# arneschneuing/DiffSBDD

Hardware: NVIDIA H100
Metric: ligand_atoms_per_sec_500step_ddpm (higher is better)
Workload: dtype f32

## Files before the change

### diffsbdd_b200/csrc/dsb_tc.cu

```cuda
#include "dsb_tc.cuh"

namespace dsb {
using namespace tc;

__global__ void pack_b_image_kernel(float* __restrict__ hi, float* __restrict__ lo, const float* __restrict__ src, int lds,
                                    int scol, int n_rows, int n_dst_off, int K, int chunks, int TN) {
  const int64_t idx = (int64_t)blockIdx.x * blockDim.x + threadIdx.x;
  if (idx >= (int64_t)n_rows * K) return;
  const int n = (int)(idx / K), k = (int)(idx - (int64_t)n * K);
  const int nd = n_dst_off + n, nt = nd / TN, nl = nd % TN;
  const int kc = k / TKC, c = (k % TKC) >> 2, j = k & 3;
  const size_t off = ((size_t)nt * chunks + kc) * (size_t)(TN * TKC) + sw128_offset(nl, c) / 4 + j;
  const float w = src[(size_t)n * lds + scol + k];
  const float h = tf32_hi(w);
  hi[off] = h;
  lo[off] = w - h;
}

void launch_pack_b_image(float* hi, float* lo, const float* src, int lds, int scol, int n_rows, int n_dst_off, int K, int tn) {
  const int64_t tot = (int64_t)n_rows * K;
  pack_b_image_kernel<<<(unsigned)((tot + 255) / 256), 256>>>(hi, lo, src, lds, scol, n_rows, n_dst_off, K, K / TKC, tn);
}

__global__ void pack_b_image_f16_kernel(__half* __restrict__ hi, __half* __restrict__ lo, const float* __restrict__ src, int lds,
                                        int scol, int n_rows, int n_dst_off, int K, int chunks, float scale, int TN) {
  const int64_t idx = (int64_t)blockIdx.x * blockDim.x + threadIdx.x;
  if (idx >= (int64_t)n_rows * K) return;
  const int n = (int)(idx / K), k = (int)(idx - (int64_t)n * K);
  const int nd = n_dst_off + n, nt = nd / TN, nl = nd % TN;
  const int kc = k / TKC16, c16 = (k % TKC16) >> 3, j = k & 7;
  const size_t off = ((size_t)nt * chunks + kc) * (size_t)(TN * 64) + sw128_offset(nl, c16) / 2 + j;
  const float w = src[(size_t)n * lds + scol + k] * scale;
  const __half h = __float2half_rn(w);
  hi[off] = h;
  lo[off] = __float2half_rn(w - __half2float(h));
}

void launch_pack_b_image_f16(float* hi, float* lo, const float* src, int lds, int scol, int n_rows, int n_dst_off, int K, float scale, int tn) {
  const int64_t tot = (int64_t)n_rows * K;
  pack_b_image_f16_kernel<<<(unsigned)((tot + 255) / 256), 256>>>(reinterpret_cast<__half*>(hi), reinterpret_cast<__half*>(lo), src,
                                                                  lds, scol, n_rows, n_dst_off, K, K / TKC16, scale, tn);
}

__global__ void absmax_kernel(const float* __restrict__ src, int lds, int scol, int n_rows, int K, unsigned* __restrict__ out) {
  const int64_t idx = (int64_t)blockIdx.x * blockDim.x + threadIdx.x;
  float v = 0.f;
  if (idx < (int64_t)n_rows * K) { const int n = (int)(idx / K), k = (int)(idx - (int64_t)n * K); v = fabsf(src[(size_t)n * lds + scol + k]); }
#pragma unroll
  for (int o = 16; o > 0; o >>= 1) v = fmaxf(v, __shfl_xor_sync(0xffffffffu, v, o));
  if ((threadIdx.x & 31) == 0) atomicMax(out, __float_as_uint(v));
}
void launch_absmax(const float* src, int lds, int scol, int n_rows, int K, unsigned* out) {
  const int64_t tot = (int64_t)n_rows * K;
  absmax_kernel<<<(unsigned)((tot + 255) / 256), 256>>>(src, lds, scol, n_rows, K, out);
}

constexpr size_t kControlBytes = 128;
static_assert(sizeof(Control) <= kControlBytes, "Control block grew");
__device__ __forceinline__ char* align1024(uint8_t* raw) {
  return reinterpret_cast<char*>(raw) + ((1024u - (smem_u32(raw) & 1023u)) & 1023u);
}
template <int H> constexpr size_t tc_smem_base() { return 1024 + (size_t)NSTAGE * Geo<H>::STAGE_BYTES + kControlBytes; }

struct TcGemmArgs {
  const float* A1; int lda1; int K1;
  const float* A2; int lda2; int K2; float div2; const int32_t* deg2;
  const float* Bhi; const float* Blo;
  const float* bias; const float* R; int ldr;
  float* C; int ldc; int M; int Nn; int act;
  float* Z; int ldz;
  int dead_mt; int dead_nt;
  float inv_scale;
};

struct TileMap {
  int ntn, ntm, dead_mt, dead_nt, nA, n_live;
  __device__ TileMap(int M, int Nn, int dmt, int dnt, int TN) {
    ntn = Nn / TN; ntm = (M + TM - 1) / TM;
    dead_nt = dnt; dead_mt = dnt > 0 ? (dmt < ntm ? dmt : ntm) : ntm;
    nA = dead_mt * ntn;
    n_live = nA + (ntm - dead_mt) * (ntn - dead_nt);
  }
  __device__ void get(int t, int& mt, int& nt) const {
    if (t < nA) { mt = t / ntn; nt = t - mt * ntn; }
    else { const int u = t - nA, w = ntn - dead_nt; mt = dead_mt + u / w; nt = dead_nt + (u - (u / w) * w); }
  }
};

template <TcFormat FMT, int H>
__global__ void __launch_bounds__(TC_THREADS, 1) tc_node_gemm_kernel(TcGemmArgs g) {
  using G = Geo<H>;
  constexpr bool F16 = FMT != TcFormat::TF32x3;
  constexpr int TN = H, HPC = F16 ? 2 : 1;
  extern __shared__ uint8_t smem_raw[];
  char* const stages = align1024(smem_raw);
  Control* ctl = reinterpret_cast<Control*>(stages + NSTAGE * G::STAGE_BYTES);
  const int wg = threadIdx.x >> 7, warp = (threadIdx.x >> 5) & 3, lane = threadIdx.x & 31;
  const TileMap tm(g.M, g.Nn, g.dead_mt, g.dead_nt, TN);
  const int n_tiles = tm.n_live;
  const int n_my = ((int)blockIdx.x < n_tiles) ? (n_tiles - (int)blockIdx.x + (int)gridDim.x - 1) / (int)gridDim.x : 0;
  if (n_my == 0) return;
  const int K = g.K1 + g.K2, chunks = K / (F16 ? TKC16 : TKC);
  const uint32_t total = (uint32_t)(n_my * chunks);
  pdl_trigger();
  if (threadIdx.x == 0) control_init(ctl);
  __syncthreads();
  pdl_wait();
  const WeightStream<FMT, H> wst{ctl, stages};
  auto issue_w = [&](uint32_t q) {
    const int it = (int)(q / chunks), kc = (int)(q - (uint32_t)it * chunks);
    int mt, nt;
    tm.get(blockIdx.x + it * gridDim.x, mt, nt);
    const size_t off = ((size_t)nt * chunks + kc) * G::B_CHUNK_FLOATS;
    wst.issue(q, g.Bhi + off, g.Blo + off);
  };
  if (threadIdx.x >= MMA_THREADS) {
    regs_dec<WEIGHT_WG_REGS>();
    if (threadIdx.x == MMA_THREADS)
      for (uint32_t q = 0; q < total; ++q) issue_w(q);
    return;
  }
  regs_inc<MMA_WG_REGS>();

  const int sr = lane >> 3, pc = lane & 7;
  const int r0 = wg * WG_ROWS + 16 * warp + 4 * sr;
  const int re = wg * WG_ROWS + 16 * warp + (lane >> 2);
  const bool divides = g.div2 != 1.0f || g.deg2 != nullptr;
  float acc[G::ACC];
  MmaTracker trk;
// ... 27 lines not shown
          }
          store_pair<FMT>(st + piece_offset<F16>(r0 + i, hf, pc), pk2(x.x, x.y), pk2(x.z, x.w));
        }
      }
      fence_proxy_async();
      wg_sync(wg);
      mbar_wait(&ctl->full_w[s], (q >> 1) & 1);
      wgmma_fence();
      mma_chunk<FMT, H>(acc, st, wg, kc == 0);
      wgmma_commit();
      trk.release_prev(ctl, (int)q, lane == 0);
    }
    trk.drain<H>(ctl, acc, lane == 0);
    const f32x2 ip = pk2(g.inv_scale, g.inv_scale);
#pragma unroll
    for (int j = 0; j < H / 8; ++j) {
      const int n = n0 + 8 * j + 2 * (lane & 3);
      const f32x2 b = g.bias ? *reinterpret_cast<const float2*>(g.bias + n) : pk2(0.f, 0.f);
#pragma unroll
      for (int hh = 0; hh < 2; ++hh) {
        f32x2 x = pk2(acc[4 * j + 2 * hh], acc[4 * j + 2 * hh + 1]);
        x = F16 ? fma2(x, ip, b) : add2(x, b);
        if (g.act == 1) x = silu2(x);
        upk2(x, acc[4 * j + 2 * hh], acc[4 * j + 2 * hh + 1]);
      }
    }
    if (g.R) {
#pragma unroll
      for (int j = 0; j < H / 8; ++j) {
        const int n = n0 + 8 * j + 2 * (lane & 3);
#pragma unroll
        for (int hh = 0; hh < 2; ++hh) {
          const int row = min(m0 + re + 8 * hh, g.M - 1);
          const f32x2 x = add2(*reinterpret_cast<const float2*>(g.R + (size_t)row * g.ldr + n),
                               pk2(acc[4 * j + 2 * hh], acc[4 * j + 2 * hh + 1]));
          upk2(x, acc[4 * j + 2 * hh], acc[4 * j + 2 * hh + 1]);
        }
      }
    }
    acc_fence(acc);
#pragma unroll
    for (int j = 0; j < H / 8; ++j) {
      const int n = n0 + 8 * j + 2 * (lane & 3);
#pragma unroll
      for (int hh = 0; hh < 2; ++hh) {
        const int row = m0 + re + 8 * hh;
        if (row < g.M) {
          *reinterpret_cast<float2*>(g.C + (size_t)row * g.ldc + n) = pk2(acc[4 * j + 2 * hh], acc[4 * j + 2 * hh + 1]);
          if (g.Z) *reinterpret_cast<float2*>(g.Z + (size_t)row * g.ldz + n) = make_float2(0.f, 0.f);
        }
      }
    }
  }
}

struct EdgeScalars {
  float d2[TM], d0[TM];
  int row[TM], col[TM], type[TM];
  float dir[3][TM];
};

template <int H>
struct EdgeExtra {
  float vec[2][3 * H];
  float wa[H];
  EdgeScalars sc[2];
};

struct TcEdgeArgs {
  const float* P; int ldp;
  const float4* x; const float4* cent; const int32_t* gid;
  const int32_t* vrow_ptr; const int32_t* vmap; int n_rows;
  const int32_t *erow, *ecol; const float* ed0; int NL;
  int nm;
  const float* W2hi[2]; const float* W2lo[2];
  const float* wr[2]; const float* wr0[2]; const float* tb[2]; const float* b2[2];
  const float* wa; const float* ba;
  float norm_constant, coords_range; int use_tanh;
  float* agg;
  float4* xagg;
  float inv_scale[2];
  float* part;
  int vcap;
};

template <bool COORD>
struct ScalarSteps {
  int e, r, c, gi;
  float d0;
  float4 xi, xj;
  __device__ __forceinline__ void step(int k, const TcEdgeArgs& a, EdgeScalars* sc, int pr, int v0, int V, int m) {
    if (k == 0) {
      const int vr = v0 + pr;
      e = a.vmap[min(vr, V - 1)];
      e = vr < V ? e : -1;
    } else if (k == 1) {
      const int ec = max(e, 0);
      r = a.erow[ec]; c = a.ecol[ec]; d0 = a.ed0[ec];
      r = e >= 0 ? r : 0; c = e >= 0 ? c : 0;
    } else if (k == 2) {
      xi = a.x[r]; xj = a.x[c];
      if (COORD) gi = a.gid[r];
    } else {
      const bool live = e >= 0;
      const float dx = xi.x - xj.x, dy = xi.y - xj.y, dz = xi.z - xj.z;
      const float d2 = dx * dx + dy * dy + dz * dz;
// ... 232 lines not shown
          t = live ? t : 0.f;
          t += __shfl_xor_sync(0xffffffffu, t, 4);
          t += __shfl_xor_sync(0xffffffffu, t, 8);
          tr[k] = t;
        }
        const int crow = hh ? crow_hi : crow_lo;
        if constexpr (DET) {
          if (chunk_lane && (lane & 3) == 0)
            reinterpret_cast<float4*>(a.part)[(size_t)((e0 + (r & ~3)) / kRowChunk) * nm + m] = make_float4(tr[0], tr[1], tr[2], 0.f);
        } else if (chunk_lane && (lane & 3) == 0 && crow >= 0) {
#pragma unroll
          for (int k = 0; k < 3; ++k) atomicAdd(reinterpret_cast<float*>(a.xagg) + (size_t)crow * 4 + k, tr[k]);
        }
      }
    }
    m = m_next; e0 = e0_next;
  }
}

template <int H> static size_t gemm_smem_bytes() { return tc_smem_base<H>(); }
template <int H> static size_t edge_smem_bytes() {
  static_assert(tc_smem_base<H>() + sizeof(EdgeExtra<H>) <= 232448, "edge kernel exceeds the 227 KB of shared memory per CTA");
  return tc_smem_base<H>() + sizeof(EdgeExtra<H>);
}

bool tc_width_supported(int H) { return H == 128 || H == 192 || H == 256; }

template <typename Fn>
static int dispatch_width(int H, Fn&& fn) {
  switch (H) {
    case 128: return fn.template operator()<128>();
    case 192: return fn.template operator()<192>();
    case 256: return fn.template operator()<256>();
    default: set_error("tensor-core kernels exist for hidden_nf 128, 192, 256 (got %d)", H); return DSB_ERR_UNSUPPORTED_CONFIG;
  }
}

template <typename Fn>
static int dispatch_tc(TcFormat f, int H, Fn&& fn) {
  return dispatch_width(H, [&]<int W>() -> int {
    switch (f) {
      case TcFormat::TF32x3: return fn.template operator()<TcFormat::TF32x3, W>();
      case TcFormat::F16x3: return fn.template operator()<TcFormat::F16x3, W>();
      default: return fn.template operator()<TcFormat::F16x1, W>();
    }
  });
}

int configure_tc_kernels(int H) {
  for (const TcFormat f : {TcFormat::TF32x3, TcFormat::F16x3, TcFormat::F16x1}) {
    const int e = dispatch_tc(f, H, [&]<TcFormat F, int W>() -> int {
      const int gs = (int)gemm_smem_bytes<W>(), es = (int)edge_smem_bytes<W>();
      DSB_CUDA_OK(cudaFuncSetAttribute(tc_node_gemm_kernel<F, W>, cudaFuncAttributeMaxDynamicSharedMemorySize, gs));
      DSB_CUDA_OK(cudaFuncSetAttribute(tc_edge_kernel<false, F, W, false>, cudaFuncAttributeMaxDynamicSharedMemorySize, es));
      DSB_CUDA_OK(cudaFuncSetAttribute(tc_edge_kernel<false, F, W, true>, cudaFuncAttributeMaxDynamicSharedMemorySize, es));
      DSB_CUDA_OK(cudaFuncSetAttribute(tc_edge_kernel<true, F, W, false>, cudaFuncAttributeMaxDynamicSharedMemorySize, es));
      DSB_CUDA_OK(cudaFuncSetAttribute(tc_edge_kernel<true, F, W, true>, cudaFuncAttributeMaxDynamicSharedMemorySize, es));
      DSB_CUDA_OK(cudaFuncSetAttribute(tc_edge_kernel<false, F, W, false, true>, cudaFuncAttributeMaxDynamicSharedMemorySize, es));
      DSB_CUDA_OK(cudaFuncSetAttribute(tc_edge_kernel<false, F, W, true, true>, cudaFuncAttributeMaxDynamicSharedMemorySize, es));
      DSB_CUDA_OK(cudaFuncSetAttribute(tc_edge_kernel<true, F, W, false, true>, cudaFuncAttributeMaxDynamicSharedMemorySize, es));
      DSB_CUDA_OK(cudaFuncSetAttribute(tc_edge_kernel<true, F, W, true, true>, cudaFuncAttributeMaxDynamicSharedMemorySize, es));
      return 0;
    });
    if (e) return e;
  }
  return 0;
}

int launch_tc_node_gemm(const dsb_dynamics* d, const GemmArgs& g, const TcImage& w, int n_tile_off, TcFormat fmt, int32_t* status,
                        cudaStream_t s) {
  (void)status;
  if (g.M == 0) return 0;
  const bool f16 = fmt != TcFormat::TF32x3;
  const int K = g.K1 + g.K2, TN = d->cfg.hidden_nf;
  if ((g.Nn % TN) || (K % TKC16) || (g.K1 % TKC16) || (g.lda1 % 4) || (g.ldc % 4)) {
    set_error("tc_node_gemm: unsupported shape K1=%d K2=%d Nn=%d", g.K1, g.K2, g.Nn);
    return DSB_ERR_INVALID_ARGUMENT;
  }
  TcGemmArgs a;
  a.A1 = g.A1; a.lda1 = g.lda1; a.K1 = g.K1; a.A2 = g.A2; a.lda2 = g.lda2; a.K2 = g.K2; a.div2 = g.div2; a.deg2 = g.deg2;
  const size_t img_off = (size_t)n_tile_off * (K / (f16 ? TKC16 : TKC)) * (size_t)(TN * TKC);
  a.Bhi = (f16 ? w.h_hi : w.t_hi) + img_off; a.Blo = (f16 ? w.h_lo : w.t_lo) + img_off;
  a.Z = g.Z; a.ldz = g.ldz;
  a.dead_nt = g.dead_cols / TN; a.dead_mt = a.dead_nt > 0 ? (g.dead_rows_from + TM - 1) / TM : 0;
  a.bias = g.bias; a.R = g.R; a.ldr = g.ldr; a.C = g.C; a.ldc = g.ldc; a.M = g.M; a.Nn = g.Nn; a.act = g.act;
  a.inv_scale = f16 ? w.h_inv : 1.0f;
  const int ntn_ = g.Nn / TN, ntm_ = (g.M + TM - 1) / TM;
  const int dmt_ = a.dead_nt > 0 ? (a.dead_mt < ntm_ ? a.dead_mt : ntm_) : ntm_;
  const int n_tiles = dmt_ * ntn_ + (ntm_ - dmt_) * (ntn_ - a.dead_nt);
  const int grid = n_tiles < d->num_sms ? n_tiles : d->num_sms;
  return dispatch_tc(fmt, TN, [&]<TcFormat F, int W>() -> int {
    DSB_CUDA_OK(launch_k(tc_node_gemm_kernel<F, W>, grid, TC_THREADS, gemm_smem_bytes<W>(), s, a));
    return 0;
  });
}

int launch_tc_edge_gcl(const dsb_dynamics* d, const Dims& dm, const Workspace& ws, const GclW& w, const float4* x, PView pv, TcFormat fmt,
                       int32_t* status, cudaStream_t s) {
  (void)status;
  const bool f16 = fmt != TcFormat::TF32x3;
  TcEdgeArgs a = {};
  a.P = pv.P; a.ldp = pv.ldp; a.x = x; a.cent = ws.cent; a.gid = ws.gid; a.vrow_ptr = ws.vrow_ptr; a.vmap = ws.vmap; a.n_rows = dm.N;
  a.erow = ws.erow; a.ecol = ws.ecol; a.ed0 = ws.ed0; a.NL = dm.NL; a.nm = 1;
  a.W2hi[0] = f16 ? w.iW2.h_hi : w.iW2.t_hi; a.W2lo[0] = f16 ? w.iW2.h_lo : w.iW2.t_lo;
  a.inv_scale[0] = f16 ? w.iW2.h_inv : 1.0f; a.inv_scale[1] = 1.0f;
  a.wr[0] = w.wr; a.wr0[0] = w.wr0; a.tb[0] = w.tb; a.b2[0] = w.b2;
  a.wa = w.wa; a.ba = w.ba; a.agg = ws.agg; a.part = ws.part; a.vcap = ws.vcap;
  const bool det = d->deterministic != 0;
  return dispatch_tc(fmt, d->cfg.hidden_nf, [&]<TcFormat F, int W>() -> int {
    auto kern = w.tb ? tc_edge_kernel<false, F, W, true> : tc_edge_kernel<false, F, W, false>;
    if (det) kern = w.tb ? tc_edge_kernel<false, F, W, true, true> : tc_edge_kernel<false, F, W, false, true>;
    DSB_CUDA_OK(launch_k(kern, d->num_sms, TC_THREADS, edge_smem_bytes<W>(), s, a));
    return 0;
  });
}

int launch_tc_edge_coord(const dsb_dynamics* d, const Dims& dm, const Workspace& ws, const EquivW& w, const float4* x, PView pv, TcFormat fmt,
                         int32_t* status, cudaStream_t s) {
  (void)status;
  const bool f16 = fmt != TcFormat::TF32x3;
  const dsb_config& c = d->cfg;
  TcEdgeArgs a = {};
  a.nm = c.reflection_equivariant ? 1 : 2;
  a.P = pv.P; a.ldp = pv.ldp; a.x = x; a.cent = ws.cent; a.gid = ws.gid; a.vrow_ptr = ws.vrow_ptr; a.vmap = ws.vmap; a.n_rows = dm.n_coord_rows;
  a.erow = ws.erow; a.ecol = ws.ecol; a.ed0 = ws.ed0; a.NL = dm.NL;
  a.inv_scale[0] = a.inv_scale[1] = 1.0f;
  for (int m = 0; m < a.nm; ++m) {
    a.W2hi[m] = f16 ? w.iW2[m].h_hi : w.iW2[m].t_hi; a.W2lo[m] = f16 ? w.iW2[m].h_lo : w.iW2[m].t_lo;
    a.inv_scale[m] = f16 ? w.iW2[m].h_inv : 1.0f;
    a.wr[m] = w.wr[m]; a.wr0[m] = w.wr0[m]; a.tb[m] = w.tb[m]; a.b2[m] = w.b2[m];
  }
  a.wa = w.w3; a.ba = nullptr;
  a.norm_constant = c.norm_constant; a.coords_range = c.coords_range; a.use_tanh = c.tanh; a.xagg = ws.xagg; a.part = ws.part; a.vcap = ws.vcap;
  const bool det = d->deterministic != 0;
  return dispatch_tc(fmt, c.hidden_nf, [&]<TcFormat F, int W>() -> int {
    auto kern = w.tb[0] ? tc_edge_kernel<true, F, W, true> : tc_edge_kernel<true, F, W, false>;
    if (det) kern = w.tb[0] ? tc_edge_kernel<true, F, W, true, true> : tc_edge_kernel<true, F, W, false, true>;
    DSB_CUDA_OK(launch_k(kern, d->num_sms, TC_THREADS, edge_smem_bytes<W>(), s, a));
    return 0;
  });
}

}
```

### diffsbdd_b200/csrc/dsb_tc.cuh

```cuda
#pragma once
#include <cuda_fp16.h>

#include "dsb_internal.cuh"
#include "dsb_wgmma.cuh"

namespace dsb {
namespace tc {

constexpr int TM = 128;
constexpr int WG_ROWS = 64;
constexpr int TKC = 32;
constexpr int TKC16 = 64;
constexpr float X_SCALE = 1.0f;
constexpr int A_CHUNK_BYTES = TM * 128;
constexpr int NSTAGE = 2;
constexpr int MMA_THREADS = 256;
constexpr int TC_THREADS = MMA_THREADS + 128;
constexpr int WEIGHT_WG_REGS = 40, MMA_WG_REGS = 232;
template <int R> __device__ __forceinline__ void regs_dec() { asm volatile("setmaxnreg.dec.sync.aligned.u32 %0;" ::"n"(R)); }
template <int R> __device__ __forceinline__ void regs_inc() { asm volatile("setmaxnreg.inc.sync.aligned.u32 %0;" ::"n"(R)); }

template <int H>
struct Geo {
  static_assert(H == 128 || H == 192 || H == 256, "tensor-core kernels are built for hidden_nf 128, 192, 256");
// ... 5 lines not shown
};

__device__ __forceinline__ uint32_t smem_u32(const void* p) { return (uint32_t)__cvta_generic_to_shared(p); }

__device__ __forceinline__ void mbar_init(uint64_t* bar, uint32_t count) {
  asm volatile("mbarrier.init.shared::cta.b64 [%0], %1;" ::"r"(smem_u32(bar)), "r"(count) : "memory");
}
__device__ __forceinline__ void mbar_arrive(uint64_t* bar) {
  asm volatile("mbarrier.arrive.shared::cta.b64 _, [%0];" ::"r"(smem_u32(bar)) : "memory");
}
__device__ __forceinline__ void mbar_arrive_expect_tx(uint64_t* bar, uint32_t bytes) {
  asm volatile("mbarrier.arrive.expect_tx.shared::cta.b64 _, [%0], %1;" ::"r"(smem_u32(bar)), "r"(bytes) : "memory");
}
__device__ __forceinline__ bool mbar_try_wait(uint64_t* bar, uint32_t parity) {
  uint32_t ok;
  asm volatile(
      "{\n\t.reg .pred P1;\n\t"
      "mbarrier.try_wait.parity.shared::cta.b64 P1, [%1], %2, %3;\n\t"
      "selp.b32 %0, 1, 0, P1;\n\t}"
      : "=r"(ok)
      : "r"(smem_u32(bar)), "r"(parity), "r"(20000u)
      : "memory");
  return ok != 0;
}
__device__ __forceinline__ void mbar_wait(uint64_t* bar, uint32_t parity) {
  uint32_t spins = 0;
  while (!mbar_try_wait(bar, parity)) {
    ++spins;
    asm volatile("{\n\t.reg .pred p;\n\tsetp.gt.u32 p, %0, %1;\n\t@p trap;\n\t}" ::"r"(spins), "r"(1u << 17));
  }
}
__device__ __forceinline__ void fence_barrier_init() { asm volatile("fence.mbarrier_init.release.cluster;" ::: "memory"); }
__device__ __forceinline__ void fence_proxy_async() { asm volatile("fence.proxy.async.shared::cta;" ::: "memory"); }
__device__ __forceinline__ void wg_sync(int wg) { asm volatile("bar.sync %0, 128;" ::"r"(wg + 1) : "memory"); }

__device__ __forceinline__ void bulk_g2s(void* smem_dst, const void* gmem_src, uint32_t bytes, uint64_t* bar) {
  asm volatile("cp.async.bulk.shared::cluster.global.mbarrier::complete_tx::bytes [%0], [%1], %2, [%3];"
               ::"r"(smem_u32(smem_dst)), "l"(gmem_src), "r"(bytes), "r"(smem_u32(bar)) : "memory");
}

__device__ __forceinline__ uint64_t wgmma_desc_sw128(uint32_t smem_addr) {
  return (uint64_t)((smem_addr >> 4) & 0x3FFFu) | (1ull << 16) | ((uint64_t)(1024 >> 4) << 32) | (1ull << 62);
}
__device__ __forceinline__ void wgmma_fence() { asm volatile("wgmma.fence.sync.aligned;" ::: "memory"); }
__device__ __forceinline__ void wgmma_commit() { asm volatile("wgmma.commit_group.sync.aligned;" ::: "memory"); }
template <int N>
__device__ __forceinline__ void wgmma_wait() { asm volatile("wgmma.wait_group.sync.aligned %0;" ::"n"(N) : "memory"); }
template <int R>
__device__ __forceinline__ void acc_fence(float (&d)[R]) {
#pragma unroll
  for (int i = 0; i < R; ++i) asm volatile("" : "+f"(d[i])::"memory");
}

template <TcFormat FMT, int H>
__device__ __forceinline__ void mma_chunk(float (&d)[H / 2], const char* st, int wg, bool first_chunk) {
  using G = Geo<H>;
  const uint32_t xhi = smem_u32(st) + (uint32_t)(wg * WG_ROWS * 128), xlo = xhi + A_CHUNK_BYTES;
  const uint32_t whi = smem_u32(st) + 2 * A_CHUNK_BYTES, wlo = whi + G::B_CHUNK_BYTES;
#pragma unroll
  for (int ks = 0; ks < 4; ++ks) {
    const uint32_t ko = ks * 32;
    const uint32_t acc = (first_chunk && ks == 0) ? 0u : 1u;
    if constexpr (FMT == TcFormat::F16x1) {
      Wgmma<H>::f16(d, wgmma_desc_sw128(xhi + ko), wgmma_desc_sw128(whi + ko), acc);
    } else if constexpr (FMT == TcFormat::F16x3) {
      Wgmma<H>::f16(d, wgmma_desc_sw128(xlo + ko), wgmma_desc_sw128(whi + ko), acc);
      Wgmma<H>::f16(d, wgmma_desc_sw128(xhi + ko), wgmma_desc_sw128(wlo + ko), 1u);
      Wgmma<H>::f16(d, wgmma_desc_sw128(xhi + ko), wgmma_desc_sw128(whi + ko), 1u);
    } else {
      Wgmma<H>::tf32(d, wgmma_desc_sw128(xlo + ko), wgmma_desc_sw128(whi + ko), acc);
      Wgmma<H>::tf32(d, wgmma_desc_sw128(xhi + ko), wgmma_desc_sw128(wlo + ko), 1u);
      Wgmma<H>::tf32(d, wgmma_desc_sw128(xhi + ko), wgmma_desc_sw128(whi + ko), 1u);
    }
  }
}

__device__ __forceinline__ float tf32_hi(float x) { return __uint_as_float((__float_as_uint(x) + 0x1000u) & 0xffffe000u); }

__device__ __host__ __forceinline__ uint32_t sw128_offset(int r, int c) {
  return (uint32_t)((r >> 3) * 1024 + (r & 7) * 128 + ((c ^ (r & 7)) << 4));
}

__device__ __forceinline__ void residual_f16(uint32_t hi2, float x0, float x1, float& r0, float& r1) {
  const __half2 h = *reinterpret_cast<const __half2*>(&hi2);
  r0 = x0 - __low2float(h);
  r1 = x1 - __high2float(h);
}
__device__ __forceinline__ uint32_t h2_bits(__half2 h) { return *reinterpret_cast<const uint32_t*>(&h); }

template <TcFormat FMT>
__device__ __forceinline__ void store_pair(char* dst, f32x2 u01, f32x2 u23) {
  float x0, x1, x2, x3;
  upk2(u01, x0, x1); upk2(u23, x2, x3);
  if constexpr (FMT == TcFormat::F16x1) {
    uint2 hv;
    hv.x = h2_bits(__floats2half2_rn(x0, x1)); hv.y = h2_bits(__floats2half2_rn(x2, x3));
    *reinterpret_cast<uint2*>(dst) = hv;
  } else if constexpr (FMT == TcFormat::F16x3) {
    const __half2 h0 = __floats2half2_rn(x0, x1), h1 = __floats2half2_rn(x2, x3);
    float l0, l1, l2, l3;
    residual_f16(h2_bits(h0), x0, x1, l0, l1); residual_f16(h2_bits(h1), x2, x3, l2, l3);
    const __half2 q0 = __floats2half2_rn(l0, l1), q1 = __floats2half2_rn(l2, l3);
    uint2 hv, lv;
    hv.x = h2_bits(h0); hv.y = h2_bits(h1);
    lv.x = h2_bits(q0); lv.y = h2_bits(q1);
    *reinterpret_cast<uint2*>(dst) = hv;
    *reinterpret_cast<uint2*>(dst + A_CHUNK_BYTES) = lv;
  } else {
    const float4 h = make_float4(tf32_hi(x0), tf32_hi(x1), tf32_hi(x2), tf32_hi(x3));
    *reinterpret_cast<float4*>(dst) = h;
    *reinterpret_cast<float4*>(dst + A_CHUNK_BYTES) = make_float4(x0 - h.x, x1 - h.y, x2 - h.z, x3 - h.w);
  }
}
template <bool F16>
__device__ __forceinline__ uint32_t piece_offset(int r, int hf, int p) {
  return F16 ? sw128_offset(r, (hf & 1) * 4 + (p >> 1)) + (uint32_t)(p & 1) * 8u : sw128_offset(r, p);
}

struct Control {
  uint64_t full_w[NSTAGE];
  uint64_t empty[NSTAGE];
};

__device__ __forceinline__ void control_init(Control* c) {
  for (int s = 0; s < NSTAGE; ++s) { mbar_init(&c->full_w[s], 1); mbar_init(&c->empty[s], 8); }
  fence_barrier_init();
}
// ... 40 lines not shown
```

### diffsbdd_b200/csrc/dsb_wgmma.cuh

```cuda
#pragma once
#include <stdint.h>

#define DSB_P10(a) "%" #a "0, %" #a "1, %" #a "2, %" #a "3, %" #a "4, %" #a "5, %" #a "6, %" #a "7, %" #a "8, %" #a "9, "
#define DSB_O8(i) "+f"(d[i]), "+f"(d[i + 1]), "+f"(d[i + 2]), "+f"(d[i + 3]), "+f"(d[i + 4]), "+f"(d[i + 5]), \
                  "+f"(d[i + 6]), "+f"(d[i + 7])

namespace dsb {
namespace tc {

template <int N> struct Wgmma;

template <> struct Wgmma<128> {
  static __device__ __forceinline__ void f16(float (&d)[64], uint64_t da, uint64_t db, uint32_t accumulate) {
    asm volatile("{\n\t.reg .pred p;\n\tsetp.ne.b32 p, %66, 0;\n\t"
                 "wgmma.mma_async.sync.aligned.m64n128k16.f32.f16.f16 {" DSB_P10() DSB_P10(1) DSB_P10(2) DSB_P10(3) DSB_P10(4) DSB_P10(5) "%60, %61, %62, %63"
                 "}, %64, %65, p, 1, 1, 0, 0;\n\t}"
                 : DSB_O8(0), DSB_O8(8), DSB_O8(16), DSB_O8(24), DSB_O8(32), DSB_O8(40), DSB_O8(48), DSB_O8(56)
                 : "l"(da), "l"(db), "r"(accumulate));
  }
  static __device__ __forceinline__ void tf32(float (&d)[64], uint64_t da, uint64_t db, uint32_t accumulate) {
    asm volatile("{\n\t.reg .pred p;\n\tsetp.ne.b32 p, %66, 0;\n\t"
                 "wgmma.mma_async.sync.aligned.m64n128k8.f32.tf32.tf32 {" DSB_P10() DSB_P10(1) DSB_P10(2) DSB_P10(3) DSB_P10(4) DSB_P10(5) "%60, %61, %62, %63"
                 "}, %64, %65, p, 1, 1;\n\t}"
                 : DSB_O8(0), DSB_O8(8), DSB_O8(16), DSB_O8(24), DSB_O8(32), DSB_O8(40), DSB_O8(48), DSB_O8(56)
                 : "l"(da), "l"(db), "r"(accumulate));
  }
};

template <> struct Wgmma<192> {
  static __device__ __forceinline__ void f16(float (&d)[96], uint64_t da, uint64_t db, uint32_t accumulate) {
    asm volatile("{\n\t.reg .pred p;\n\tsetp.ne.b32 p, %98, 0;\n\t"
                 "wgmma.mma_async.sync.aligned.m64n192k16.f32.f16.f16 {" DSB_P10() DSB_P10(1) DSB_P10(2) DSB_P10(3) DSB_P10(4) DSB_P10(5) DSB_P10(6) DSB_P10(7) DSB_P10(8) "%90, %91, %92, %93, %94, %95"
                 "}, %96, %97, p, 1, 1, 0, 0;\n\t}"
                 : DSB_O8(0), DSB_O8(8), DSB_O8(16), DSB_O8(24), DSB_O8(32), DSB_O8(40), DSB_O8(48), DSB_O8(56), DSB_O8(64), DSB_O8(72), DSB_O8(80), DSB_O8(88)
                 : "l"(da), "l"(db), "r"(accumulate));
  }
  static __device__ __forceinline__ void tf32(float (&d)[96], uint64_t da, uint64_t db, uint32_t accumulate) {
    asm volatile("{\n\t.reg .pred p;\n\tsetp.ne.b32 p, %98, 0;\n\t"
                 "wgmma.mma_async.sync.aligned.m64n192k8.f32.tf32.tf32 {" DSB_P10() DSB_P10(1) DSB_P10(2) DSB_P10(3) DSB_P10(4) DSB_P10(5) DSB_P10(6) DSB_P10(7) DSB_P10(8) "%90, %91, %92, %93, %94, %95"
                 "}, %96, %97, p, 1, 1;\n\t}"
                 : DSB_O8(0), DSB_O8(8), DSB_O8(16), DSB_O8(24), DSB_O8(32), DSB_O8(40), DSB_O8(48), DSB_O8(56), DSB_O8(64), DSB_O8(72), DSB_O8(80), DSB_O8(88)
                 : "l"(da), "l"(db), "r"(accumulate));
  }
};

template <> struct Wgmma<256> {
  static __device__ __forceinline__ void f16(float (&d)[128], uint64_t da, uint64_t db, uint32_t accumulate) {
    asm volatile("{\n\t.reg .pred p;\n\tsetp.ne.b32 p, %130, 0;\n\t"
                 "wgmma.mma_async.sync.aligned.m64n256k16.f32.f16.f16 {" DSB_P10() DSB_P10(1) DSB_P10(2) DSB_P10(3) DSB_P10(4) DSB_P10(5) DSB_P10(6) DSB_P10(7) DSB_P10(8) DSB_P10(9) DSB_P10(10) DSB_P10(11) "%120, %121, %122, %123, %124, %125, %126, %127"
                 "}, %128, %129, p, 1, 1, 0, 0;\n\t}"
                 : DSB_O8(0), DSB_O8(8), DSB_O8(16), DSB_O8(24), DSB_O8(32), DSB_O8(40), DSB_O8(48), DSB_O8(56), DSB_O8(64), DSB_O8(72), DSB_O8(80), DSB_O8(88), DSB_O8(96), DSB_O8(104), DSB_O8(112), DSB_O8(120)
                 : "l"(da), "l"(db), "r"(accumulate));
  }
  static __device__ __forceinline__ void tf32(float (&d)[128], uint64_t da, uint64_t db, uint32_t accumulate) {
    asm volatile("{\n\t.reg .pred p;\n\tsetp.ne.b32 p, %130, 0;\n\t"
                 "wgmma.mma_async.sync.aligned.m64n256k8.f32.tf32.tf32 {" DSB_P10() DSB_P10(1) DSB_P10(2) DSB_P10(3) DSB_P10(4) DSB_P10(5) DSB_P10(6) DSB_P10(7) DSB_P10(8) DSB_P10(9) DSB_P10(10) DSB_P10(11) "%120, %121, %122, %123, %124, %125, %126, %127"
                 "}, %128, %129, p, 1, 1;\n\t}"
                 : DSB_O8(0), DSB_O8(8), DSB_O8(16), DSB_O8(24), DSB_O8(32), DSB_O8(40), DSB_O8(48), DSB_O8(56), DSB_O8(64), DSB_O8(72), DSB_O8(80), DSB_O8(88), DSB_O8(96), DSB_O8(104), DSB_O8(112), DSB_O8(120)
                 : "l"(da), "l"(db), "r"(accumulate));
  }
};
}
}
// ... 4 lines not shown
```

### profiles/node_gemm_breakdown.py

```python
from __future__ import annotations

import argparse
import json
import os
import statistics
import subprocess
import sys

import torch

ROOT = os.path.dirname(os.path.dirname(os.path.abspath(__file__)))
sys.path.insert(0, ROOT)

import bench
from diffsbdd_b200 import synthetic as syn
from diffsbdd_b200.dynamics import EGNNDynamics

TM = 128
PEAK_TFLOPS = {'3xfp16': 989.0, '3xtf32': 495.0}
HBM_TBS = 3.35


def gpu_info():
    try:
        out = subprocess.run(['nvidia-smi', '--id=0', '--query-gpu=name,power.limit,clocks.sm,clocks.max.sm',
                              '--format=csv,noheader'], capture_output=True, text=True, timeout=30).stdout.strip()
        return out
    except Exception:
        return None


def launch_plan(cfg, n, n_lig):
    H = cfg.hidden_nf
    nm = 1 if cfg.reflection_equivariant else 2
    conditional = not cfg.update_pocket_coords
    plan = []
    for layer in range(cfg.n_layers):
        for sub in range(cfg.inv_sublayers):
            if not (sub == 0 and layer > 0):
                plan.append(('g1', H, 2 * H, False, False, 0, 0))
            plan.append(('g2', 2 * H, H, False, False, 0, 0))
            plan.append(('g3', H, H, True, True, 0, 0))
        plan.append(('g4', H, nm * 2 * H + 2 * H, False, False, n_lig if conditional else 0, nm * H if conditional else 0))
    return plan


def shape_counts(H, M, K, Nn, has_r, has_z, dead_from, dead_cols, f16, n_sms):
    ntn, ntm = Nn // H, (M + TM - 1) // TM
    dnt = dead_cols // H
    dmt = min((dead_from + TM - 1) // TM, ntm) if dnt > 0 else ntm
    tiles = dmt * ntn + (ntm - dmt) * (ntn - dnt)
    chunks = K // (64 if f16 else 32)
    dead_rows = max(M - dmt * TM, 0) if dnt > 0 else 0
    c_elems = M * Nn - dead_rows * dnt * H
    hbm = 4 * (M * K + (M * Nn if has_r else 0) + c_elems + (M * H if has_z else 0))
    return {'tiles': tiles, 'ctas': min(tiles, n_sms), 'chunks_per_tile': chunks,
            'exec_gflop': 6.0 * tiles * TM * H * K / 1e9, 'hbm_lb_mb': hbm / 1e6,
            'l2_weight_mb': tiles * chunks * 2 * H * 128 / 1e6}


def profile_workload(name, calls, warmup, math_mode, flush):
    a = argparse.Namespace(workload=name)
    cfg, _, _, _ = bench.workload(a)
    _, B, NL, NP, _, _, _, _ = bench.WORKLOADS[name]
    sd = syn.synthetic_state_dict(cfg, 0)
    dyn = EGNNDynamics.from_config(cfg, device='cuda')
    dyn.load_state_dict(sd)
    dyn.eval()
    dyn.math_mode = math_mode
    inp = [x.cuda() for x in syn.synthetic_denoiser_inputs(cfg, [NL] * B, [NP] * B, seed=1)]
    H, M = cfg.hidden_nf, B * (NL + NP)
    plan = launch_plan(cfg, M, B * NL)
    with torch.no_grad():
        for _ in range(warmup):
            bench.l2_flush(flush)
            dyn(*inp)
        torch.cuda.synchronize()
        with torch.profiler.profile(activities=[torch.profiler.ProfilerActivity.CUDA]) as prof:
            for _ in range(calls):
                bench.l2_flush(flush)
                dyn(*inp)
            torch.cuda.synchronize()
    raw = sorted(((e.start_ns(), e.start_ns() + e.duration_ns(), e.name()) for e in prof.profiler.kineto_results.events()
                  if e.device_type() == torch.autograd.DeviceType.CUDA), key=lambda t: t[0])
    kern, last_end = [], 0
    for s, e, n in raw:
        kern.append((s, max(e - max(s, last_end), 0), n, e - s))
        last_end = max(last_end, e)
    gemms = [k for k in kern if 'tc_node_gemm_kernel' in k[2]]
    if len(gemms) != calls * len(plan):
        raise SystemExit(f'{name}: {len(gemms)} node-GEMM kernels for {calls} calls, expected {len(plan)} per call')
    per_label, span = {}, {}
    for i, (_, dur, _, sp) in enumerate(gemms):
        per_label.setdefault(plan[i % len(plan)][0], []).append(dur / 1e3)
        span.setdefault(plan[i % len(plan)][0], []).append(sp / 1e3)
    classes = {'node_gemm': 'tc_node_gemm_kernel', 'edge_gcl': 'tc_edge_kernel<false', 'edge_coord': 'tc_edge_kernel<true'}
    by_class = {c: round(sum(d for _, d, n, _ in kern if key in n) / 1e6 / calls, 4) for c, key in classes.items()}
    by_class['all_dsb_kernels'] = round(sum(d for _, d, n, _ in kern if 'dsb::' in n) / 1e6 / calls, 4)
    f16 = math_mode == '3xfp16'
    rows = []
    for lab in ('g1', 'g2', 'g3', 'g4'):
        if lab not in per_label:
            continue
        p = next(x for x in plan if x[0] == lab)
        sc = shape_counts(H, M, p[1], p[2], p[3], p[4], p[5], p[6], f16, torch.cuda.get_device_properties(0).multi_processor_count)
        us = statistics.median(per_label[lab])
        rows.append({'label': lab, 'launches_per_call': len(per_label[lab]) // calls, 'M': M, 'K': p[1], 'Nn': p[2],
                     'us_median': round(us, 2), 'us_min': round(min(per_label[lab]), 2), 'us_max': round(max(per_label[lab]), 2),
                     'span_us_median': round(statistics.median(span[lab]), 2),
                     **sc, 'exec_tflops': round(sc['exec_gflop'] / us * 1e3, 1),
                     'tensor_bound_us': round(sc['exec_gflop'] / PEAK_TFLOPS[math_mode] / 1e-3, 2),
                     'hbm_bound_us': round(sc['hbm_lb_mb'] / HBM_TBS, 2),
                     'l2_weight_gbs': round(sc['l2_weight_mb'] / us * 1e3, 1)})
    node_ms = sum(r['us_median'] * r['launches_per_call'] for r in rows) / 1e3
    return {'workload': name, 'hidden_nf': H, 'M': M, 'math_mode': math_mode, 'calls': calls,
            'node_gemm_ms_per_call_from_medians': round(node_ms, 4), 'ms_per_call_by_class': by_class, 'per_label': rows}


def print_table(res):
    print(f"\n{res['workload']} (H = {res['hidden_nf']}, M = {res['M']}, {res['math_mode']}); per call: {res['ms_per_call_by_class']}")
    print('| launch | per call | us/launch (min-max) | span us | tiles | CTAs | exec TFLOP/s | tensor bound us | HBM LB MB | HBM bound us '
          '| L2 weight MB | L2 weight GB/s |')
    print('|---|---|---|---|---|---|---|---|---|---|---|---|')
    for r in res['per_label']:
        print(f"| {r['label']} | {r['launches_per_call']} | {r['us_median']} ({r['us_min']}-{r['us_max']}) | {r['span_us_median']} | {r['tiles']} | {r['ctas']} "
              f"| {r['exec_tflops']} | {r['tensor_bound_us']} | {r['hbm_lb_mb']:.1f} | {r['hbm_bound_us']} | {r['l2_weight_mb']:.1f} "
              f"| {r['l2_weight_gbs']} |")


def main():
    ap = argparse.ArgumentParser()
    ap.add_argument('--workloads', default='fullatom,moad,moad_ca')
    ap.add_argument('--calls', type=int, default=20)
    ap.add_argument('--warmup', type=int, default=5)
    ap.add_argument('--math-mode', default='3xfp16', choices=sorted(PEAK_TFLOPS))
    ap.add_argument('--out', default=None)
    args = ap.parse_args()
    if not torch.cuda.is_available():
        raise SystemExit('node_gemm_breakdown.py needs a CUDA device')
    flush = torch.zeros(64 * 1024 * 1024, dtype=torch.float32, device='cuda')
    out = {'gpu': gpu_info(), 'torch_device': torch.cuda.get_device_name(0), 'results': []}
    print('gpu (name, power limit, SM clock, max SM clock):', out['gpu'])
    for w in args.workloads.split(','):
        res = profile_workload(w, args.calls, args.warmup, args.math_mode, flush)
        out['results'].append(res)
        print_table(res)
    print('\n(tensor / HBM bounds: data-sheet peaks of a 700 W H100 SXM, not measured; DRAM traffic is not measured)')
    if args.out:
        with open(args.out, 'w') as f:
            json.dump(out, f, indent=1)


if __name__ == '__main__':
    main()
```

Before: 966.8.

## Add half-width N-slice node GEMM kernel with resident A tile for fp16

Adds a node GEMM kernel for fp16 formats in the plain K=H, no-activation, no-A2 case. It splits each output tile into two half-width N slices, doubling the work units so more SMs get used when tiles are few. The A tile stays resident in shared memory across consecutive slices of the same M tile, and the epilogue of one slice overlaps the MMAs of the next. It adds m64n64 and m64n96 wgmma wrappers. The cost is that weight-slice and A-build work is repeated across CTAs that share an M tile, and the dispatch logic is more complex.

Result: faster. 980.2 (median of 6 runs) (+1.4%).

```diff
diff --git a/diffsbdd_b200/csrc/dsb_tc.cu b/diffsbdd_b200/csrc/dsb_tc.cu
--- a/diffsbdd_b200/csrc/dsb_tc.cu
+++ b/diffsbdd_b200/csrc/dsb_tc.cu
@@ -75,6 +75,7 @@
 
 struct TileMap {
   int ntn, ntm, dead_mt, dead_nt, nA, n_live;
+  TileMap() = default;
   __device__ TileMap(int M, int Nn, int dmt, int dnt, int TN) {
     ntn = Nn / TN; ntm = (M + TM - 1) / TM;
     dead_nt = dnt; dead_mt = dnt > 0 ? (dmt < ntm ? dmt : ntm) : ntm;
@@ -208,6 +209,200 @@
       }
     }
   }
+}
+
+constexpr int SLICE_STAGES = 3;
+struct SliceControl {
+  uint64_t full_w[SLICE_STAGES];
+  uint64_t empty[SLICE_STAGES];
+};
+static_assert(sizeof(SliceControl) <= kControlBytes, "SliceControl grew");
+
+template <TcFormat FMT, int H>
+struct SliceGeo {
+  static_assert(FMT != TcFormat::TF32x3, "the resident A tile is built for the fp16 formats");
+  static constexpr int NPROD = FMT == TcFormat::F16x1 ? 1 : 2;
+  static constexpr int HS = H / 2;
+  static constexpr int CHUNKS = H / TKC16;
+  static constexpr int A_STRIDE = NPROD * A_CHUNK_BYTES;
+  static constexpr int W_BYTES = HS * 128;
+  static constexpr int STAGE_BYTES = NPROD * W_BYTES;
+  static constexpr size_t SMEM = 1024 + (size_t)CHUNKS * A_STRIDE + (size_t)SLICE_STAGES * STAGE_BYTES + kControlBytes;
+  static_assert(SMEM <= 232448, "slice node GEMM exceeds the 227 KB of shared memory per CTA");
+};
+
+template <TcFormat FMT, int H>
+__global__ void __launch_bounds__(TC_THREADS, 1) tc_node_gemm_slices_kernel(TcGemmArgs g) {
+  using SG = SliceGeo<FMT, H>;
+  constexpr int HS = SG::HS, CH = SG::CHUNKS, NS = SLICE_STAGES;
+  extern __shared__ uint8_t smem_raw[];
+  char* const a_tile = align1024(smem_raw);
+  char* const ring = a_tile + CH * SG::A_STRIDE;
+  SliceControl* ctl = reinterpret_cast<SliceControl*>(ring + NS * SG::STAGE_BYTES);
+  const int wg = threadIdx.x >> 7, warp = (threadIdx.x >> 5) & 3, lane = threadIdx.x & 31;
+  pdl_trigger();
+  if (threadIdx.x == 0) {
+    for (int s = 0; s < NS; ++s) { mbar_init(&ctl->full_w[s], 1); mbar_init(&ctl->empty[s], 8); }
+    fence_barrier_init();
+  }
+  __syncthreads();
+  pdl_wait();
+  auto slice_range = [&](TileMap& tm, int& s_begin, int& s_end) {
+    tm = TileMap(g.M, g.Nn, g.dead_mt, g.dead_nt, H);
+    s_begin = (int)((int64_t)blockIdx.x * (2 * tm.n_live) / gridDim.x);
+    s_end = (int)((int64_t)(blockIdx.x + 1) * (2 * tm.n_live) / gridDim.x);
+  };
+  if (threadIdx.x >= MMA_THREADS) {
+    regs_dec<WEIGHT_WG_REGS>();
+    if (threadIdx.x == MMA_THREADS) {
+      TileMap tm;
+      int s_begin, s_end;
+      slice_range(tm, s_begin, s_end);
+      uint32_t q = 0;
+      for (int s = s_begin; s < s_end; ++s) {
+        int mt, nt;
+        tm.get(s >> 1, mt, nt);
+        const size_t off = (size_t)nt * CH * Geo<H>::B_CHUNK_FLOATS + (size_t)(s & 1) * (SG::W_BYTES / 4);
+        for (int kc = 0; kc < CH; ++kc, ++q) {
+          const int st = (int)(q % NS);
+          if (q >= NS) mbar_wait(&ctl->empty[st], (q / NS - 1) & 1);
+          char* dst = ring + st * SG::STAGE_BYTES;
+          const size_t o = off + (size_t)kc * Geo<H>::B_CHUNK_FLOATS;
+          mbar_arrive_expect_tx(&ctl->full_w[st], SG::STAGE_BYTES);
+          bulk_g2s(dst, g.Bhi + o, SG::W_BYTES, &ctl->full_w[st]);
+          if constexpr (SG::NPROD == 2) bulk_g2s(dst + SG::W_BYTES, g.Blo + o, SG::W_BYTES, &ctl->full_w[st]);
+        }
+      }
+    }
+    return;
+  }
+  regs_inc<MMA_WG_REGS>();
+  TileMap tm;
+  int s_begin, s_end;
+  slice_range(tm, s_begin, s_end);
+
+  const int sr = lane >> 3, pc = lane & 7;
+  const int r0 = wg * WG_ROWS + 16 * warp + 4 * sr;
+  const int re = wg * WG_ROWS + 16 * warp + (lane >> 2);
+  const bool leader = lane == 0;
+  const uint32_t a_wg = smem_u32(a_tile) + (uint32_t)(wg * WG_ROWS * 128), ring_u32 = smem_u32(ring);
+  float acc0[HS / 2], acc1[HS / 2];
+  uint32_t q = 0, rel = 0;
+  int a_m0 = -1;
+  int pm0 = 0, pn0 = 0;
+
+  auto release_to = [&](uint32_t upto) {
+#pragma unroll
+    for (int i = 0; i < 2; ++i) {
+      const bool p = rel < upto;
+      if (leader && p) mbar_arrive(&ctl->empty[rel % NS]);
+      rel += p ? 1u : 0u;
+    }
+  };
+  auto build = [&](int m0, int kc) {
+    int r = r0, p = pc;
+    asm volatile("" : "+r"(r), "+r"(p));
+    const float* src = g.A1 + (size_t)(m0 + r) * g.lda1 + kc * TKC16 + 4 * p;
+    char* const dst = a_tile + kc * SG::A_STRIDE;
+#pragma unroll
+    for (int h = 0; h < 2; ++h) {
+      float4 v[4];
+#pragma unroll
+      for (int i = 0; i < 4; ++i) {
+        v[i] = make_float4(0.f, 0.f, 0.f, 0.f);
+        if (m0 + r + i < g.M) v[i] = *reinterpret_cast<const float4*>(src + (size_t)i * g.lda1 + h * TKC);
+      }
+#pragma unroll
+      for (int i = 0; i < 4; ++i)
+        store_pair<FMT>(dst + piece_offset<true>(r + i, h, p), pk2(v[i].x, v[i].y), pk2(v[i].z, v[i].w));
+    }
+  };
+  auto epilogue = [&](float (&d)[HS / 2], int m0, int n0) {
+    const f32x2 ip = pk2(g.inv_scale, g.inv_scale);
+#pragma unroll
+    for (int j = 0; j < HS / 8; ++j) {
+      const int n = n0 + 8 * j + 2 * (lane & 3);
+      const f32x2 b = g.bias ? *reinterpret_cast<const float2*>(g.bias + n) : pk2(0.f, 0.f);
+#pragma unroll
+      for (int hh = 0; hh < 2; ++hh)
+        upk2(fma2(pk2(d[4 * j + 2 * hh], d[4 * j + 2 * hh + 1]), ip, b), d[4 * j + 2 * hh], d[4 * j + 2 * hh + 1]);
+    }
+    if (g.R) {
+#pragma unroll
+      for (int j = 0; j < HS / 8; ++j) {
+        const int n = n0 + 8 * j + 2 * (lane & 3);
+#pragma unroll
+        for (int hh = 0; hh < 2; ++hh) {
+          const int row = min(m0 + re + 8 * hh, g.M - 1);
+          const f32x2 x = add2(*reinterpret_cast<const float2*>(g.R + (size_t)row * g.ldr + n),
+                               pk2(d[4 * j + 2 * hh], d[4 * j + 2 * hh + 1]));
+          upk2(x, d[4 * j + 2 * hh], d[4 * j + 2 * hh + 1]);
+        }
+      }
+    }
+    acc_fence(d);
+#pragma unroll
+    for (int j = 0; j < HS / 8; ++j) {
+      const int n = n0 + 8 * j + 2 * (lane & 3);
+#pragma unroll
+      for (int hh = 0; hh < 2; ++hh) {
+        const int row = m0 + re + 8 * hh;
+        if (row < g.M) {
+          *reinterpret_cast<float2*>(g.C + (size_t)row * g.ldc + n) = pk2(d[4 * j + 2 * hh], d[4 * j + 2 * hh + 1]);
+          if (g.Z) *reinterpret_cast<float2*>(g.Z + (size_t)row * g.ldz + n) = make_float2(0.f, 0.f);
+        }
+      }
+    }
+  };
+  auto slice = [&](float (&d)[HS / 2], float (&dp)[HS / 2], int s, bool has_prev) {
+    int mt, nt;
+    tm.get(s >> 1, mt, nt);
+    const int m0 = mt * TM, n0 = nt * H + (s & 1) * HS;
+    const bool build_a = m0 != a_m0;
+    if (build_a && has_prev) { wgmma_wait<0>(); release_to(q); }
+    a_m0 = m0;
+#pragma unroll
+    for (int kc = 0; kc < CH; ++kc) {
+      if (build_a) {
+        build(m0, kc);
+        fence_proxy_async();
+        wg_sync(wg);
+      }
+      const int st = (int)(q % NS);
+      mbar_wait(&ctl->full_w[st], (q / NS) & 1);
+      wgmma_fence();
+      uint32_t xa = a_wg + kc * SG::A_STRIDE;
+      asm volatile("" : "+r"(xa));
+      const uint32_t wa = ring_u32 + st * SG::STAGE_BYTES;
+      mma_k_chunk<FMT, HS>(d, xa, xa + A_CHUNK_BYTES, wa, wa + SG::W_BYTES, kc == 0);
+      wgmma_commit();
+      ++q;
+      if (kc == 1) {
+        if (has_prev) epilogue(dp, pm0, pn0);
+      } else {
+        wgmma_wait<1>();
+        release_to(q - 1);
+        if (kc == 0) acc_fence(dp);
+      }
+    }
+    pm0 = m0; pn0 = n0;
+  };
+
+  int s = s_begin;
+  slice(acc0, acc1, s, false);
+  while (++s < s_end) {
+    slice(acc1, acc0, s, true);
+    if (++s == s_end) {
+      wgmma_wait<0>();
+      acc_fence(acc1);
+      epilogue(acc1, pm0, pn0);
+      return;
+    }
+    slice(acc0, acc1, s, true);
+  }
+  wgmma_wait<0>();
+  acc_fence(acc0);
+  epilogue(acc0, pm0, pn0);
 }
 
 struct EdgeScalars {
@@ -546,6 +741,9 @@
     const int e = dispatch_tc(f, H, [&]<TcFormat F, int W>() -> int {
       const int gs = (int)gemm_smem_bytes<W>(), es = (int)edge_smem_bytes<W>();
       DSB_CUDA_OK(cudaFuncSetAttribute(tc_node_gemm_kernel<F, W>, cudaFuncAttributeMaxDynamicSharedMemorySize, gs));
+      if constexpr (F != TcFormat::TF32x3)
+        DSB_CUDA_OK(cudaFuncSetAttribute(tc_node_gemm_slices_kernel<F, W>, cudaFuncAttributeMaxDynamicSharedMemorySize,
+                                         (int)SliceGeo<F, W>::SMEM));
       DSB_CUDA_OK(cudaFuncSetAttribute(tc_edge_kernel<false, F, W, false>, cudaFuncAttributeMaxDynamicSharedMemorySize, es));
       DSB_CUDA_OK(cudaFuncSetAttribute(tc_edge_kernel<false, F, W, true>, cudaFuncAttributeMaxDynamicSharedMemorySize, es));
       DSB_CUDA_OK(cudaFuncSetAttribute(tc_edge_kernel<true, F, W, false>, cudaFuncAttributeMaxDynamicSharedMemorySize, es));
@@ -582,8 +780,16 @@
   const int ntn_ = g.Nn / TN, ntm_ = (g.M + TM - 1) / TM;
   const int dmt_ = a.dead_nt > 0 ? (a.dead_mt < ntm_ ? a.dead_mt : ntm_) : ntm_;
   const int n_tiles = dmt_ * ntn_ + (ntm_ - dmt_) * (ntn_ - a.dead_nt);
-  const int grid = n_tiles < d->num_sms ? n_tiles : d->num_sms;
+  const bool slices = f16 && g.K1 == TN && g.K2 == 0 && g.act == 0;
+  const int units = slices ? 2 * n_tiles : n_tiles;
+  const int grid = units < d->num_sms ? units : d->num_sms;
   return dispatch_tc(fmt, TN, [&]<TcFormat F, int W>() -> int {
+    if constexpr (F != TcFormat::TF32x3) {
+      if (slices) {
+        DSB_CUDA_OK(launch_k(tc_node_gemm_slices_kernel<F, W>, grid, TC_THREADS, SliceGeo<F, W>::SMEM, s, a));
+        return 0;
+      }
+    }
     DSB_CUDA_OK(launch_k(tc_node_gemm_kernel<F, W>, grid, TC_THREADS, gemm_smem_bytes<W>(), s, a));
     return 0;
   });
diff --git a/diffsbdd_b200/csrc/dsb_tc.cuh b/diffsbdd_b200/csrc/dsb_tc.cuh
--- a/diffsbdd_b200/csrc/dsb_tc.cuh
+++ b/diffsbdd_b200/csrc/dsb_tc.cuh
@@ -81,27 +81,32 @@
   for (int i = 0; i < R; ++i) asm volatile("" : "+f"(d[i])::"memory");
 }
 
-template <TcFormat FMT, int H>
-__device__ __forceinline__ void mma_chunk(float (&d)[H / 2], const char* st, int wg, bool first_chunk) {
-  using G = Geo<H>;
-  const uint32_t xhi = smem_u32(st) + (uint32_t)(wg * WG_ROWS * 128), xlo = xhi + A_CHUNK_BYTES;
-  const uint32_t whi = smem_u32(st) + 2 * A_CHUNK_BYTES, wlo = whi + G::B_CHUNK_BYTES;
+template <TcFormat FMT, int N>
+__device__ __forceinline__ void mma_k_chunk(float (&d)[N / 2], uint32_t xhi, uint32_t xlo, uint32_t whi, uint32_t wlo,
+                                            bool first_chunk) {
 #pragma unroll
   for (int ks = 0; ks < 4; ++ks) {
     const uint32_t ko = ks * 32;
     const uint32_t acc = (first_chunk && ks == 0) ? 0u : 1u;
     if constexpr (FMT == TcFormat::F16x1) {
-      Wgmma<H>::f16(d, wgmma_desc_sw128(xhi + ko), wgmma_desc_sw128(whi + ko), acc);
+      Wgmma<N>::f16(d, wgmma_desc_sw128(xhi + ko), wgmma_desc_sw128(whi + ko), acc);
     } else if constexpr (FMT == TcFormat::F16x3) {
-      Wgmma<H>::f16(d, wgmma_desc_sw128(xlo + ko), wgmma_desc_sw128(whi + ko), acc);
-      Wgmma<H>::f16(d, wgmma_desc_sw128(xhi + ko), wgmma_desc_sw128(wlo + ko), 1u);
-      Wgmma<H>::f16(d, wgmma_desc_sw128(xhi + ko), wgmma_desc_sw128(whi + ko), 1u);
+      Wgmma<N>::f16(d, wgmma_desc_sw128(xlo + ko), wgmma_desc_sw128(whi + ko), acc);
+      Wgmma<N>::f16(d, wgmma_desc_sw128(xhi + ko), wgmma_desc_sw128(wlo + ko), 1u);
+      Wgmma<N>::f16(d, wgmma_desc_sw128(xhi + ko), wgmma_desc_sw128(whi + ko), 1u);
     } else {
-      Wgmma<H>::tf32(d, wgmma_desc_sw128(xlo + ko), wgmma_desc_sw128(whi + ko), acc);
-      Wgmma<H>::tf32(d, wgmma_desc_sw128(xhi + ko), wgmma_desc_sw128(wlo + ko), 1u);
-      Wgmma<H>::tf32(d, wgmma_desc_sw128(xhi + ko), wgmma_desc_sw128(whi + ko), 1u);
+      Wgmma<N>::tf32(d, wgmma_desc_sw128(xlo + ko), wgmma_desc_sw128(whi + ko), acc);
+      Wgmma<N>::tf32(d, wgmma_desc_sw128(xhi + ko), wgmma_desc_sw128(wlo + ko), 1u);
+      Wgmma<N>::tf32(d, wgmma_desc_sw128(xhi + ko), wgmma_desc_sw128(whi + ko), 1u);
     }
   }
+}
+
+template <TcFormat FMT, int H>
+__device__ __forceinline__ void mma_chunk(float (&d)[H / 2], const char* st, int wg, bool first_chunk) {
+  using G = Geo<H>;
+  const uint32_t xhi = smem_u32(st) + (uint32_t)(wg * WG_ROWS * 128), whi = smem_u32(st) + 2 * A_CHUNK_BYTES;
+  mma_k_chunk<FMT, H>(d, xhi, xhi + A_CHUNK_BYTES, whi, whi + G::B_CHUNK_BYTES, first_chunk);
 }
 
 __device__ __forceinline__ float tf32_hi(float x) { return __uint_as_float((__float_as_uint(x) + 0x1000u) & 0xffffe000u); }
diff --git a/diffsbdd_b200/csrc/dsb_wgmma.cuh b/diffsbdd_b200/csrc/dsb_wgmma.cuh
--- a/diffsbdd_b200/csrc/dsb_wgmma.cuh
+++ b/diffsbdd_b200/csrc/dsb_wgmma.cuh
@@ -9,6 +9,26 @@
 namespace tc {
 
 template <int N> struct Wgmma;
+
+template <> struct Wgmma<64> {
+  static __device__ __forceinline__ void f16(float (&d)[32], uint64_t da, uint64_t db, uint32_t accumulate) {
+    asm volatile("{\n\t.reg .pred p;\n\tsetp.ne.b32 p, %34, 0;\n\t"
+                 "wgmma.mma_async.sync.aligned.m64n64k16.f32.f16.f16 {" DSB_P10() DSB_P10(1) DSB_P10(2) "%30, %31"
+                 "}, %32, %33, p, 1, 1, 0, 0;\n\t}"
+                 : DSB_O8(0), DSB_O8(8), DSB_O8(16), DSB_O8(24)
+                 : "l"(da), "l"(db), "r"(accumulate));
+  }
+};
+
+template <> struct Wgmma<96> {
+  static __device__ __forceinline__ void f16(float (&d)[48], uint64_t da, uint64_t db, uint32_t accumulate) {
+    asm volatile("{\n\t.reg .pred p;\n\tsetp.ne.b32 p, %50, 0;\n\t"
+                 "wgmma.mma_async.sync.aligned.m64n96k16.f32.f16.f16 {" DSB_P10() DSB_P10(1) DSB_P10(2) DSB_P10(3) "%40, %41, %42, %43, %44, %45, %46, %47"
+                 "}, %48, %49, p, 1, 1, 0, 0;\n\t}"
+                 : DSB_O8(0), DSB_O8(8), DSB_O8(16), DSB_O8(24), DSB_O8(32), DSB_O8(40)
+                 : "l"(da), "l"(db), "r"(accumulate));
+  }
+};
 
 template <> struct Wgmma<128> {
   static __device__ __forceinline__ void f16(float (&d)[64], uint64_t da, uint64_t db, uint32_t accumulate) {
diff --git a/profiles/node_gemm_breakdown.py b/profiles/node_gemm_breakdown.py
--- a/profiles/node_gemm_breakdown.py
+++ b/profiles/node_gemm_breakdown.py
@@ -45,7 +45,7 @@
     return plan
 
 
-def shape_counts(H, M, K, Nn, has_r, has_z, dead_from, dead_cols, f16, n_sms):
+def shape_counts(H, M, K, Nn, has_r, has_z, dead_from, dead_cols, f16, n_sms, slices):
     ntn, ntm = Nn // H, (M + TM - 1) // TM
     dnt = dead_cols // H
     dmt = min((dead_from + TM - 1) // TM, ntm) if dnt > 0 else ntm
@@ -54,7 +54,7 @@
     dead_rows = max(M - dmt * TM, 0) if dnt > 0 else 0
     c_elems = M * Nn - dead_rows * dnt * H
     hbm = 4 * (M * K + (M * Nn if has_r else 0) + c_elems + (M * H if has_z else 0))
-    return {'tiles': tiles, 'ctas': min(tiles, n_sms), 'chunks_per_tile': chunks,
+    return {'tiles': tiles, 'ctas': min(2 * tiles if slices else tiles, n_sms), 'chunks_per_tile': chunks,
             'exec_gflop': 6.0 * tiles * TM * H * K / 1e9, 'hbm_lb_mb': hbm / 1e6,
             'l2_weight_mb': tiles * chunks * 2 * H * 128 / 1e6}
 
@@ -87,14 +87,15 @@
     for s, e, n in raw:
         kern.append((s, max(e - max(s, last_end), 0), n, e - s))
         last_end = max(last_end, e)
-    gemms = [k for k in kern if 'tc_node_gemm_kernel' in k[2]]
+    gemms = [k for k in kern if 'tc_node_gemm_' in k[2]]
     if len(gemms) != calls * len(plan):
         raise SystemExit(f'{name}: {len(gemms)} node-GEMM kernels for {calls} calls, expected {len(plan)} per call')
-    per_label, span = {}, {}
-    for i, (_, dur, _, sp) in enumerate(gemms):
+    per_label, span, kernel = {}, {}, {}
+    for i, (_, dur, kname, sp) in enumerate(gemms):
         per_label.setdefault(plan[i % len(plan)][0], []).append(dur / 1e3)
         span.setdefault(plan[i % len(plan)][0], []).append(sp / 1e3)
-    classes = {'node_gemm': 'tc_node_gemm_kernel', 'edge_gcl': 'tc_edge_kernel<false', 'edge_coord': 'tc_edge_kernel<true'}
+        kernel[plan[i % len(plan)][0]] = 'tc_node_gemm_slices_kernel' if 'slices' in kname else 'tc_node_gemm_kernel'
+    classes = {'node_gemm': 'tc_node_gemm_', 'edge_gcl': 'tc_edge_kernel<false', 'edge_coord': 'tc_edge_kernel<true'}
     by_class = {c: round(sum(d for _, d, n, _ in kern if key in n) / 1e6 / calls, 4) for c, key in classes.items()}
     by_class['all_dsb_kernels'] = round(sum(d for _, d, n, _ in kern if 'dsb::' in n) / 1e6 / calls, 4)
     f16 = math_mode == '3xfp16'
@@ -103,9 +104,10 @@
         if lab not in per_label:
             continue
         p = next(x for x in plan if x[0] == lab)
-        sc = shape_counts(H, M, p[1], p[2], p[3], p[4], p[5], p[6], f16, torch.cuda.get_device_properties(0).multi_processor_count)
+        sc = shape_counts(H, M, p[1], p[2], p[3], p[4], p[5], p[6], f16, torch.cuda.get_device_properties(0).multi_processor_count,
+                          kernel[lab] == 'tc_node_gemm_slices_kernel')
         us = statistics.median(per_label[lab])
-        rows.append({'label': lab, 'launches_per_call': len(per_label[lab]) // calls, 'M': M, 'K': p[1], 'Nn': p[2],
+        rows.append({'label': lab, 'kernel': kernel[lab], 'launches_per_call': len(per_label[lab]) // calls, 'M': M, 'K': p[1], 'Nn': p[2],
                      'us_median': round(us, 2), 'us_min': round(min(per_label[lab]), 2), 'us_max': round(max(per_label[lab]), 2),
                      'span_us_median': round(statistics.median(span[lab]), 2),
                      **sc, 'exec_tflops': round(sc['exec_gflop'] / us * 1e3, 1),
@@ -119,11 +121,11 @@
 
 def print_table(res):
     print(f"\n{res['workload']} (H = {res['hidden_nf']}, M = {res['M']}, {res['math_mode']}); per call: {res['ms_per_call_by_class']}")
-    print('| launch | per call | us/launch (min-max) | span us | tiles | CTAs | exec TFLOP/s | tensor bound us | HBM LB MB | HBM bound us '
-          '| L2 weight MB | L2 weight GB/s |')
-    print('|---|---|---|---|---|---|---|---|---|---|---|---|')
+    print('| launch | kernel | per call | us/launch (min-max) | span us | tiles | CTAs | exec TFLOP/s | tensor bound us | HBM LB MB '
+          '| HBM bound us | L2 weight MB | L2 weight GB/s |')
+    print('|---|---|---|---|---|---|---|---|---|---|---|---|---|')
     for r in res['per_label']:
-        print(f"| {r['label']} | {r['launches_per_call']} | {r['us_median']} ({r['us_min']}-{r['us_max']}) | {r['span_us_median']} | {r['tiles']} | {r['ctas']} "
+        print(f"| {r['label']} | {r['kernel']} | {r['launches_per_call']} | {r['us_median']} ({r['us_min']}-{r['us_max']}) | {r['span_us_median']} | {r['tiles']} | {r['ctas']} "
               f"| {r['exec_tflops']} | {r['tensor_bound_us']} | {r['hbm_lb_mb']:.1f} | {r['hbm_bound_us']} | {r['l2_weight_mb']:.1f} "
               f"| {r['l2_weight_gbs']} |")
 
```
